# kristi700/ViT-SSL

Hardware: AMD Instinct MI355X
Metric: images_per_sec (higher is better)
Workload: dtype bf16; 1 GPU; ViT-B/16 SimMIM 224x224 mask 0.6 dropout 0.1 AdamW, batch 256/GPU; global_batch=256, parallelism=dp1

## Files before the change

__graft_entry__.py:

```python
import os
import subprocess
import sys
from concurrent.futures import ThreadPoolExecutor

ROOT = os.path.dirname(os.path.abspath(__file__))
PKG = os.path.join(ROOT, "vit-ssl_amd")
CSRC = os.path.join(PKG, "csrc")
OUT_DIR = os.path.join(PKG, "vitssl_hip")
LIB = os.path.join(OUT_DIR, "libvitssl_hip.so")
SOURCES = ["error.cpp", "gemm_nt.hip", "gemm_tn.hip", "layernorm.hip", "attention.hip", "attention_long.hip", "elementwise.hip", "dino.hip", "augment.hip", "transforms.hip", "metrics.hip", "classify.hip", "fp8.hip"]
HIPCC = os.environ.get("HIPCC", "/opt/rocm/bin/hipcc")
PER_FILE_FLAGS = {"augment.hip": ["-ffp-contract=off"], "transforms.hip": ["-ffp-contract=off"]}
FLAGS = ["--offload-arch=gfx950", "-O3", "-fPIC", "-std=c++17", "-Wno-unused-result"] + os.environ.get("VITSSL_HIPCC_FLAGS", "").split()


def _needs_rebuild(target, deps):
    if not os.path.exists(target):
        return True
    t = os.path.getmtime(target)
    return any(os.path.getmtime(d) > t for d in deps if os.path.exists(d))


def build(force: bool = False, verbose: bool = False) -> None:
    srcs = [os.path.join(CSRC, s) for s in SOURCES if os.path.exists(os.path.join(CSRC, s))]
    hdrs = [os.path.join(CSRC, "common.h"), os.path.join(CSRC, "attention_tiles.h"), os.path.join(CSRC, "attention_bwd.h"),
            os.path.join(CSRC, "resample_taps.h"),
            os.path.join(ROOT, "include", "vitssl_hip.h"), os.path.join(ROOT, "include", "vitssl_transforms.h"),
            os.path.join(ROOT, "include", "vitssl_metrics.h"), os.path.join(ROOT, "include", "vitssl_classify.h")]
    objdir = os.path.join(CSRC, "build")
    os.makedirs(objdir, exist_ok=True)

    def compile_one(src):
        obj = os.path.join(objdir, os.path.basename(src) + ".o")
        if force or _needs_rebuild(obj, [src] + hdrs + [os.path.abspath(__file__)]):
            cmd = [HIPCC] + FLAGS + PER_FILE_FLAGS.get(os.path.basename(src), []) + ["-x", "hip", "-c", src, "-o", obj]
            r = subprocess.run(cmd, capture_output=True, text=True)
            if r.returncode != 0:
                raise RuntimeError(f"hipcc failed for {src}:\n{r.stderr[-4000:]}")
            if verbose and r.stderr.strip():
                print(r.stderr, file=sys.stderr)
        return obj

    with ThreadPoolExecutor(max_workers=4) as ex:
        objs = list(ex.map(compile_one, srcs))
    if force or _needs_rebuild(LIB, objs):
        cmd = [HIPCC, "--offload-arch=gfx950", "-shared", "-fPIC", "-o", LIB] + objs
        r = subprocess.run(cmd, capture_output=True, text=True)
        if r.returncode != 0:
            raise RuntimeError(f"link failed:\n{r.stderr[-4000:]}")
    if PKG not in sys.path:
        sys.path.insert(0, PKG)
    import vitssl_hip
    vitssl_hip.lib()


def smoke() -> None:
    for p in (ROOT, PKG):
        if p not in sys.path:
            sys.path.insert(0, p)
    import torch
    from vitssl_hip import smoke_check
# ... 8 lines not shown
```

vit-ssl_amd/csrc/elementwise.hip:

```cpp
#include "common.h"

namespace {

constexpr int EW_THREADS = 256;

inline unsigned ew_grid(long long work_items) {
  long long g = (work_items + EW_THREADS - 1) / EW_THREADS;
  if (g < 1) g = 1;
  return (unsigned)g;
}

__global__ void dropout_mask_kernel(unsigned char* keep, long long ngroups, DropKey dk) {
  const long long grp = (long long)blockIdx.x * blockDim.x + threadIdx.x;
  if (grp >= ngroups) return;
  float m[4];
  drop_mult4(dk, (unsigned)grp, m);
  uchar4 o;
  o.x = m[0] != 0.f; o.y = m[1] != 0.f; o.z = m[2] != 0.f; o.w = m[3] != 0.f;
  if (dk.thr == 0) o = make_uchar4(1, 1, 1, 1);
  *(uchar4*)(keep + 4 * grp) = o;
}

template <bool GATHER, typename OutT>
__global__ void patchify_kernel(const float* __restrict__ img, const int* __restrict__ idx, OutT* __restrict__ out,
                                long long nrows, int C, int H, int W, int P) {
  const int gw = W / P, gh = H / P;
  const int pd4 = C * P * P / 4;
  const long long t = (long long)blockIdx.x * blockDim.x + threadIdx.x;
  if (t >= nrows * pd4) return;
  const long long r = t / pd4;
  const int f = (int)(t - r * pd4) * 4;
  const long long m = GATHER ? (long long)idx[r] : r;
  const long long b = m / (gh * gw);
  const int pi = (int)(m - b * gh * gw);
  const int py = pi / gw, px = pi - py * gw;
  const int c = f / (P * P);
  const int kh = (f - c * P * P) / P;
  const int kw = f - c * P * P - kh * P;
  const f32x4 v = *(const f32x4*)(img + ((b * C + c) * H + (py * P + kh)) * (long long)W + px * P + kw);
  if constexpr (sizeof(OutT) == 2) {
    u32x2 w = {pack_bf2(v[0], v[1]), pack_bf2(v[2], v[3])};
    *(u32x2*)((bf16_t*)out + r * (4LL * pd4) + f) = w;
  } else {
    *(f32x4*)((float*)out + r * (4LL * pd4) + f) = v;
  }
}

__global__ void gather_rows_bf16_kernel(const float* __restrict__ x, const int* __restrict__ idx, bf16_t* __restrict__ out,
                                        int n_idx, int cols) {
  const int c4n = cols >> 2;
  const long long t = (long long)blockIdx.x * blockDim.x + threadIdx.x;
  if (t >= (long long)n_idx * c4n) return;
  const int i = (int)(t / c4n);
  const int c = (int)(t - (long long)i * c4n) * 4;
  const f32x4 v = *(const f32x4*)(x + (long long)idx[i] * cols + c);
  u32x2 w = {pack_bf2(v[0], v[1]), pack_bf2(v[2], v[3])};
  *(u32x2*)(out + (long long)i * cols + c) = w;
}

__global__ void scatter_rows_f32_kernel(const bf16_t* __restrict__ src, const int* __restrict__ inv, float* __restrict__ g,
                                        long long rows, int cols) {
  const int c4n = cols >> 2;
  const long long t = (long long)blockIdx.x * blockDim.x + threadIdx.x;
  if (t >= rows * c4n) return;
  const long long r = t / c4n;
  const int c = (int)(t - r * c4n) * 4;
  const int i = inv[r];
  f32x4 v = {0.f, 0.f, 0.f, 0.f};
  if (i >= 0) {
    const u32x2 w = *(const u32x2*)(src + (long long)i * cols + c);
    v = f32x4{bf_lo(w[0]), bf_hi(w[0]), bf_lo(w[1]), bf_hi(w[1])};
  }
  *(f32x4*)(g + r * cols + c) = v;
}

__global__ void gather_cls_kernel(const float* __restrict__ x, float* __restrict__ out, int B, int T, int D) {
  const int d4n = D >> 2;
  const long long t = (long long)blockIdx.x * blockDim.x + threadIdx.x;
  if (t >= (long long)B * d4n) return;
  const int b = (int)(t / d4n);
// ... 125 lines not shown
__global__ void cast_bf16_kernel(const float* __restrict__ src, bf16_t* __restrict__ dst, long long n) {
  const long long n4 = n >> 2;
  for (long long i = (long long)blockIdx.x * blockDim.x + threadIdx.x; i < n4; i += (long long)gridDim.x * blockDim.x) {
    const f32x4 v = *(const f32x4*)(src + 4 * i);
    u32x2 w = {pack_bf2(v[0], v[1]), pack_bf2(v[2], v[3])};
    *(u32x2*)(dst + 4 * i) = w;
  }
  if (blockIdx.x == 0 && threadIdx.x < (n & 3)) dst[(n4 << 2) + threadIdx.x] = f2bf(src[(n4 << 2) + threadIdx.x]);
}

__global__ void cast_transpose_kernel(const float* __restrict__ src, bf16_t* __restrict__ dst, bf16_t* __restrict__ dst_t,
                                      int R, int C) {
  __shared__ bf16_t tile[64][66];
  const int r0 = blockIdx.y * 64, c0 = blockIdx.x * 64;
  const int tx = threadIdx.x & 63, ty = threadIdx.x >> 6;
  for (int rr = ty; rr < 64; rr += 4) {
    const int r = r0 + rr, c = c0 + tx;
    bf16_t h = 0;
    if (r < R && c < C) {
      h = f2bf(src[(long long)r * C + c]);
      if (dst) dst[(long long)r * C + c] = h;
    }
    tile[rr][tx] = h;
  }
  __syncthreads();
  if (dst_t) {
    for (int cc = ty; cc < 64; cc += 4) {
      const int c = c0 + cc, r = r0 + tx;
      if (c < C && r < R) dst_t[(long long)c * R + r] = tile[tx][cc];
    }
  }
}

__global__ void cast_transpose_batch_kernel(const vitssl_cast_job_t* __restrict__ jobs, const int* __restrict__ tile_start,
                                            int njobs) {
  __shared__ bf16_t tile[64][66];
  const int b = blockIdx.x;
  int lo = 0, hi = njobs;
  while (hi - lo > 1) {
    const int mid = (lo + hi) >> 1;
    if (tile_start[mid] <= b) lo = mid; else hi = mid;
  }
  const vitssl_cast_job_t j = jobs[lo];
  const int t = b - tile_start[lo];
  const int tx_n = (j.C + 63) >> 6;
  const int r0 = (t / tx_n) * 64, c0 = (t % tx_n) * 64;
  const int R = j.R, C = j.C;
  bf16_t* dst = (bf16_t*)j.dst;
  bf16_t* dst_t = (bf16_t*)j.dst_t;
  const int tx = threadIdx.x & 63, ty = threadIdx.x >> 6;
  for (int rr = ty; rr < 64; rr += 4) {
    const int r = r0 + rr, c = c0 + tx;
    bf16_t h = 0;
    if (r < R && c < C) {
      h = f2bf(j.src[(long long)r * C + c]);
      if (dst) dst[(long long)r * C + c] = h;
    }
    tile[rr][tx] = h;
  }
  __syncthreads();
  if (dst_t) {
    for (int cc = ty; cc < 64; cc += 4) {
      const int c = c0 + cc, r = r0 + tx;
      if (c < C && r < R) dst_t[(long long)c * R + r] = tile[tx][cc];
    }
  }
}

__global__ void adamw_kernel(float* __restrict__ p, const float* __restrict__ g, float* __restrict__ m, float* __restrict__ v,
                             long long n, float lr, float b1, float b2, float eps, float wd, float bc1, float bc2_sqrt,
                             float gscale) {
  const long long n4 = n >> 2;
  const float step_size = lr / bc1;
  for (long long i = (long long)blockIdx.x * blockDim.x + threadIdx.x; i < n4; i += (long long)gridDim.x * blockDim.x) {
    f32x4 pv = *(const f32x4*)(p + 4 * i);
    const f32x4 gv = *(const f32x4*)(g + 4 * i) * gscale;
    f32x4 mv = *(const f32x4*)(m + 4 * i);
    f32x4 vv = *(const f32x4*)(v + 4 * i);
    pv *= (1.f - lr * wd);
    mv = mv * b1 + gv * (1.f - b1);
    vv = vv * b2 + gv * gv * (1.f - b2);
#pragma unroll
// ... 130 lines not shown
  VS_CHECK_ARG(keep && rows > 0 && cols > 0 && cols % 4 == 0, "dropout_mask: cols must be a multiple of 4");
  VS_CHECK_ARG((unsigned long long)rows * (unsigned long long)cols < (1ull << 34), "dropout_mask: the stream's group counter is 32 bits (rows * cols < 2^34)");
  const long long ng = rows * cols / 4;
  hipLaunchKernelGGL(dropout_mask_kernel, dim3(ew_grid(ng)), dim3(EW_THREADS), 0, (hipStream_t)stream, keep, ng, make_drop_key(d));
  VS_CHECK_LAUNCH("dropout_mask");
  return VITSSL_OK;
}

static int check_patch_args(const char* who, int B, int C, int H, int W, int P) {
  VS_CHECK_ARG(B > 0 && C > 0 && P > 0 && P % 4 == 0, "%s: patch size %d must be a positive multiple of 4", who, P);
  VS_CHECK_ARG(H % P == 0 && W % P == 0, "%s: image %dx%d not divisible by patch %d", who, H, W, P);
  return VITSSL_OK;
}

extern "C" int vitssl_patchify_bf16(const float* img, void* patches, int B, int C, int H, int W, int P, void* stream) {
  VS_CHECK_ARG(img && patches, "patchify: null pointer");
  if (int rc = check_patch_args("patchify", B, C, H, W, P)) return rc;
  const long long nrows = (long long)B * (H / P) * (W / P);
  const long long work = nrows * (C * P * P / 4);
  hipLaunchKernelGGL((patchify_kernel<false, bf16_t>), dim3(ew_grid(work)), dim3(EW_THREADS), 0, (hipStream_t)stream, img,
                     (const int*)nullptr, (bf16_t*)patches, nrows, C, H, W, P);
  VS_CHECK_LAUNCH("patchify");
  return VITSSL_OK;
}

extern "C" int vitssl_gather_patches_f32(const float* img, const int32_t* idx, float* out, int n_idx, int C, int H, int W,
                                         int P, void* stream) {
  VS_CHECK_ARG(img && idx && out && n_idx > 0, "gather_patches: null pointer / empty");
  if (int rc = check_patch_args("gather_patches", 1, C, H, W, P)) return rc;
  const long long work = (long long)n_idx * (C * P * P / 4);
  hipLaunchKernelGGL((patchify_kernel<true, float>), dim3(ew_grid(work)), dim3(EW_THREADS), 0, (hipStream_t)stream, img, idx,
                     out, (long long)n_idx, C, H, W, P);
  VS_CHECK_LAUNCH("gather_patches");
  return VITSSL_OK;
}

extern "C" int vitssl_gather_rows_bf16(const float* x, const int32_t* idx, void* out, int n_idx, int cols, void* stream) {
  VS_CHECK_ARG(x && idx && out && n_idx > 0 && cols > 0 && cols % 4 == 0, "gather_rows: bad args");
  hipLaunchKernelGGL(gather_rows_bf16_kernel, dim3(ew_grid((long long)n_idx * (cols / 4))), dim3(EW_THREADS), 0,
                     (hipStream_t)stream, x, idx, (bf16_t*)out, n_idx, cols);
  VS_CHECK_LAUNCH("gather_rows");
  return VITSSL_OK;
}

extern "C" int vitssl_scatter_rows_f32(const void* src_bf16, const int32_t* inv, float* g, int64_t rows, int cols, void* stream) {
  VS_CHECK_ARG(src_bf16 && inv && g && rows > 0 && cols > 0 && cols % 4 == 0, "scatter_rows: bad args");
  hipLaunchKernelGGL(scatter_rows_f32_kernel, dim3(ew_grid(rows * (cols / 4))), dim3(EW_THREADS), 0, (hipStream_t)stream,
                     (const bf16_t*)src_bf16, inv, g, (long long)rows, cols);
  VS_CHECK_LAUNCH("scatter_rows");
  return VITSSL_OK;
}

extern "C" int vitssl_gather_cls_f32(const float* x, float* out, int B, int T, int D, void* stream) {
  VS_CHECK_ARG(x && out && B > 0 && T > 0 && D > 0 && D % 4 == 0, "gather_cls: bad args");
  hipLaunchKernelGGL(gather_cls_kernel, dim3(ew_grid((long long)B * (D / 4))), dim3(EW_THREADS), 0, (hipStream_t)stream, x, out, B, T, D);
  VS_CHECK_LAUNCH("gather_cls");
  return VITSSL_OK;
}

extern "C" int vitssl_scatter_cls_f32(const float* gcls, float* g, int B, int T, int D, void* stream) {
  VS_CHECK_ARG(gcls && g && B > 0 && T > 0 && D > 0 && D % 4 == 0, "scatter_cls: bad args");
  hipLaunchKernelGGL(scatter_cls_kernel, dim3(ew_grid((long long)B * T * (D / 4))), dim3(EW_THREADS), 0, (hipStream_t)stream, gcls, g, B, T, D);
  VS_CHECK_LAUNCH("scatter_cls");
  return VITSSL_OK;
}

// ... 71 lines not shown
}

extern "C" int vitssl_colsum_bf16(const void* x_bf16, float* out, int64_t rows, int cols, float* workspace, int64_t workspace_floats,
                                  void* stream) {
  VS_CHECK_ARG(x_bf16 && out && rows > 0 && cols > 0 && cols % 4 == 0, "colsum_bf16: bad args");
  int splits = (int)((rows + 127) / 128);
  if (splits > 512) splits = 512;
  float* parts = vs_sum_parts(workspace, workspace_floats, (long long)splits * cols, rows, cols, "colsum_bf16");
  if (!parts) return VITSSL_ERR_ARG;
  hipLaunchKernelGGL(colsum_bf16_kernel, dim3((cols / 4 + EW_THREADS - 1) / EW_THREADS, splits), dim3(EW_THREADS), 0,
                     (hipStream_t)stream, (const bf16_t*)x_bf16, parts, (long long)rows, cols);
  VS_CHECK_LAUNCH("colsum_bf16");
  return vs_reduce_parts(out, parts, splits, cols, cols, (hipStream_t)stream);
}

extern "C" int vitssl_cast_bf16(const float* src, void* dst, int64_t n, void* stream) {
  VS_CHECK_ARG(src && dst && n > 0, "cast_bf16: bad args");
  hipLaunchKernelGGL(cast_bf16_kernel, dim3(stream_grid(n / 4)), dim3(EW_THREADS), 0, (hipStream_t)stream, src, (bf16_t*)dst, (long long)n);
  VS_CHECK_LAUNCH("cast_bf16");
  return VITSSL_OK;
}

extern "C" int vitssl_cast_transpose_bf16(const float* src, void* dst, void* dst_t, int R, int C, void* stream) {
  VS_CHECK_ARG(src && (dst || dst_t) && R > 0 && C > 0, "cast_transpose: bad args");
  hipLaunchKernelGGL(cast_transpose_kernel, dim3((C + 63) / 64, (R + 63) / 64), dim3(EW_THREADS), 0, (hipStream_t)stream, src,
                     (bf16_t*)dst, (bf16_t*)dst_t, R, C);
  VS_CHECK_LAUNCH("cast_transpose");
  return VITSSL_OK;
}

extern "C" int vitssl_cast_transpose_batch(const vitssl_cast_job_t* jobs, const int* tile_start, int njobs, int total_tiles,
                                           void* stream) {
  VS_CHECK_ARG(jobs && tile_start && njobs > 0 && total_tiles > 0, "cast_transpose_batch: bad args");
  hipLaunchKernelGGL(cast_transpose_batch_kernel, dim3(total_tiles), dim3(EW_THREADS), 0, (hipStream_t)stream, jobs, tile_start,
                     njobs);
  VS_CHECK_LAUNCH("cast_transpose_batch");
  return VITSSL_OK;
}

extern "C" int vitssl_adamw(float* p, const float* g, float* m, float* v, int64_t n, float lr, float beta1, float beta2,
                            float eps, float wd, int step, float gscale, void* stream) {
  VS_CHECK_ARG(p && g && m && v && n > 0 && step >= 1, "adamw: bad args");
  const double bc1 = 1.0 - pow((double)beta1, (double)step);
  const double bc2 = 1.0 - pow((double)beta2, (double)step);
  hipLaunchKernelGGL(adamw_kernel, dim3(stream_grid(n / 4)), dim3(EW_THREADS), 0, (hipStream_t)stream, p, g, m, v, (long long)n, lr,
                     beta1, beta2, eps, wd, (float)bc1, (float)sqrt(bc2), gscale);
  VS_CHECK_LAUNCH("adamw");
  return VITSSL_OK;
}

extern "C" int vitssl_ema(float* teacher, const float* student, int64_t n, float m, void* stream) {
  VS_CHECK_ARG(teacher && student && n > 0, "ema: bad args");
  hipLaunchKernelGGL(ema_kernel, dim3(stream_grid(n / 4)), dim3(EW_THREADS), 0, (hipStream_t)stream, teacher, student, (long long)n, m);
  VS_CHECK_LAUNCH("ema");
  return VITSSL_OK;
}
```

vit-ssl_amd/vit_core/ssl/simmim/model.py:

```python
import torch
from torch import nn
from torch.autograd import Function

from ... import _runtime as R
from ..._runtime import BF16, F32, L, ops
from ...encoder_block import EncoderBlock
from .masking import draw_mask, mask_indices_np


class _SimMIMRuntime:

    def __init__(self, model: "SimMIMViT", device):
        self.model = model
        self.device = device
        C, H, W = model.input_shape
        self.P = model.patch_size
        self.C, self.H, self.W = C, H, W
        self.N = (H // self.P) * (W // self.P)
        self.Pd = C * self.P * self.P
        self.D = model.embed_dim
        self.store = R.FlatStore(model, device)
        st = self.store
        prefixes = [f"encoder_blocks.{i}." for i in range(len(model.encoder_blocks))]
        self.stack = R.EncoderStack(st, prefixes, self.D, model.num_heads, model.mlp_dim, model.dropout_p)
        st.register_weight("proj", lambda: st.view("projection.weight", (self.D, self.Pd)), transposed_too=False)
        st.register_weight("head", lambda: st.view("simmim_head.weight", (self.Pd, self.D)))
        self.ws = R.Workspace()
        self.rec = None
        self.save_gen = 0

    def valid_for(self, device) -> bool:
        return device == self.device and self.store.is_attached()

    def embed(self, x, mask_d, tag=""):
        st, ws = self.store, self.ws
        B = x.shape[0]
        M = B * self.N
        patches = ws.get(tag + "patches", (M, self.Pd), BF16, x.device)
        ops.patchify_bf16(x, patches, self.P)
        x0 = ws.get(tag + "x0", (M, self.D), F32, x.device)
        ops.gemm_nt(patches, st.w("proj"), x0, L.EPI_EMBED, bias=st.view("projection.bias"),
                    embed=(mask_d, st.view("mask_token") if mask_d is not None else None,
                           st.view("positional_embedding", (self.N, self.D)), self.N, self.N, 0))
        return x0, patches

    def prepare_mask(self, mask_cpu, dev):
        idx, inv, mflat = mask_indices_np(mask_cpu.contiguous())
        M, Mm = inv.size, idx.size
        key = (M, Mm, str(dev))
        if getattr(self, "_stage_key", None) != key:
            nslots = 4
            self._stage = [dict(idx=torch.empty(Mm, dtype=torch.int32).pin_memory(),
                                inv=torch.empty(M, dtype=torch.int32).pin_memory(),
                                mask=torch.empty(M, dtype=torch.uint8).pin_memory(), ev=None) for _ in range(nslots)]
            self._stage_dev = [dict(idx=torch.empty(Mm, dtype=torch.int32, device=dev),
                                    inv=torch.empty(M, dtype=torch.int32, device=dev),
                                    mask=torch.empty(M, dtype=torch.uint8, device=dev)) for _ in range(nslots)]
            self._stage_pos = 0
            self._stage_key = key
        k = self._stage_pos % len(self._stage)
        self._stage_pos += 1
        slot, d = self._stage[k], self._stage_dev[k]
        if slot["ev"] is not None:
            slot["ev"].synchronize()
        slot["idx"].numpy()[:] = idx
        slot["inv"].numpy()[:] = inv
        slot["mask"].numpy()[:] = mflat
        for name in ("idx", "inv", "mask"):
            d[name].copy_(slot[name], non_blocking=True)
        slot["ev"] = torch.cuda.Event()
        slot["ev"].record(torch.cuda.current_stream())
        return d["idx"], d["inv"], d["mask"]

    def forward(self, x, training: bool, save: bool, mask_cpu=None, prepared=None):
        st, ws = self.store, self.ws
        if x.dim() != 4 or tuple(x.shape[1:]) != (self.C, self.H, self.W):
            raise L.VitsslError(f"SimMIMViT: expected input [B,{self.C},{self.H},{self.W}], got {tuple(x.shape)}")
        self.stack.check_tokens(self.N)
        x = R.as_f32(x)
        B = x.shape[0]
        M = B * self.N
        st.refresh_weights()
        dev = x.device
        if prepared is None:
            if mask_cpu is None:
                mask_cpu = draw_mask(B, self.N, self.model.mask_ratio)
            prepared = self.prepare_mask(mask_cpu, dev)
        seed = R.next_seed() if (training and self.stack.p > 0) else 0
        idx_d, inv_d, mask_d = prepared
        Mm = idx_d.numel()

        targets = torch.empty(Mm, self.Pd, dtype=F32, device=dev)
        if Mm == 0:
            if save:
                self.save_gen += 1
                self.rec = dict(B=B, M=M, Mm=0)
            return torch.empty(0, self.Pd, dtype=F32, device=dev), targets, mask_d.view(B, self.N, 1).bool()
        ops.gather_patches_f32(x, idx_d, targets, self.P)
        tag = "" if save else "tmp."
        x0, patches = self.embed(x, mask_d, tag)
        xL, _ = self.stack.forward(x0, B, self.N, training, seed, save=save, slot="a")
        sel = ws.get(tag + "sel", (Mm, self.D), BF16, dev)
        ops.gather_rows_bf16(xL, idx_d, sel)
        pred = torch.empty(Mm, self.Pd, dtype=F32, device=dev)
        ops.gemm_nt(sel, st.w("head"), pred, L.EPI_F32, bias=st.view("simmim_head.bias"))
        if save:
            self.save_gen += 1
            self.rec = dict(B=B, M=M, Mm=Mm, idx=idx_d, inv=inv_d, mask=mask_d, patches=patches, sel=sel)
        return pred, targets, mask_d.view(B, self.N, 1).bool()

    def backward(self, dpred_bf16, reducer=None):
        st, ws, rec = self.store, self.ws, self.rec
        B, M, Mm = rec["B"], rec["M"], rec["Mm"]
        if Mm == 0:
            if reducer is not None:
                reducer.ready(0, st.gflat.numel())
            return
        dev = dpred_bf16.device
        gv = st.gview
        ops.colsum_bf16(dpred_bf16, gv("simmim_head.bias"))
        ops.gemm_tn(dpred_bf16, rec["sel"], gv("simmim_head.weight", (self.Pd, self.D)))
        dsel = ws.get("dsel", (Mm, self.D), BF16, dev)
        ops.gemm_nt(dpred_bf16, st.w("head.T"), dsel, L.EPI_BF16)
        g = ws.get("g", (M, self.D), F32, dev)
        ops.scatter_rows_f32(dsel, rec["inv"], g)
        if reducer is not None:
            reducer.ready(*st.span("simmim_head.weight", "simmim_head.bias"))
        g = self.stack.backward(g, slot="a", reducer=reducer)
        dproj = ws.get("dproj", (M, self.D), BF16, dev)
        ops.embed_bwd(g, rec["mask"], dproj, gv("positional_embedding", (self.N, self.D)), gv("mask_token"),
                      gv("projection.bias"), None, B, self.N, 0, self.D)
        ops.gemm_tn(dproj, rec["patches"], gv("projection.weight", (self.D, self.Pd)))
        if reducer is not None:
# ... 126 lines not shown
```

vit-ssl_amd/vitssl_hip/_lib.py:

```python
import ctypes as C
import os
import re

_HERE = os.path.dirname(os.path.abspath(__file__))
LIB_PATH = os.environ.get("VITSSL_LIB") or os.path.join(_HERE, "libvitssl_hip.so")
HEADER_PATH = os.path.normpath(os.path.join(_HERE, "..", "..", "include", "vitssl_hip.h"))
TRANSFORMS_HEADER_PATH = os.path.normpath(os.path.join(_HERE, "..", "..", "include", "vitssl_transforms.h"))
METRICS_HEADER_PATH = os.path.normpath(os.path.join(_HERE, "..", "..", "include", "vitssl_metrics.h"))
CLASSIFY_HEADER_PATH = os.path.normpath(os.path.join(_HERE, "..", "..", "include", "vitssl_classify.h"))


class VitsslError(RuntimeError):
    pass


class Dropout(C.Structure):
    _fields_ = [("p", C.c_float), ("site", C.c_uint32), ("seed", C.c_uint64)]


class Embed(C.Structure):
    _fields_ = [("mask", C.c_void_p), ("mask_token", C.c_void_p), ("pos", C.c_void_p),
                ("tokens", C.c_int), ("out_tokens", C.c_int), ("tok_offset", C.c_int)]


class TnJob(C.Structure):
    _fields_ = [("A", C.c_void_p), ("B", C.c_void_p), ("C", C.c_void_p), ("N1", C.c_int), ("N2", C.c_int)]


class Fp8TnJob(C.Structure):
    _fields_ = [("A8", C.c_void_p), ("B8", C.c_void_p), ("C", C.c_void_p), ("N1", C.c_int), ("N2", C.c_int),
                ("alpha", C.c_void_p), ("alpha2", C.c_void_p)]


class Gemm(C.Structure):
    _fields_ = [("A", C.c_void_p), ("B", C.c_void_p), ("M", C.c_int64), ("N", C.c_int), ("K", C.c_int),
                ("epilogue", C.c_int), ("bias", C.c_void_p), ("aux", C.c_void_p), ("out0", C.c_void_p),
                ("out1", C.c_void_p), ("colsum", C.c_void_p), ("drop", Dropout), ("embed", Embed),
                ("workspace", C.c_void_p), ("workspace_floats", C.c_int64)]


class Fp8Gemm(C.Structure):
# ... 41 lines not shown
    "vitssl_cast_bf16": [_vp, _vp, _i64, _vp],
    "vitssl_cast_transpose_bf16": [_vp, _vp, _vp, _i, _i, _vp],
    "vitssl_cast_transpose_batch": [_vp, _vp, _i, _i, _vp],
    "vitssl_bicubic_resize_fwd": [_vp, _vp, _i, _i, _i, _i, _i, _vp],
    "vitssl_bicubic_resize_bwd": [_vp, _vp, _i, _i, _i, _i, _i, _vp],
    "vitssl_aug_resized_crop_u8": [_vp, _vp, _vp, _vp, _i, _i, _i, _i, _vp],
    "vitssl_aug_color_u8": [_vp, _vp, _vp, _i, _i, _vp],
    "vitssl_aug_blur_to_tensor": [_vp, _vp, _vp, _i, _i, _i, _vp],
    "vitssl_adamw": [_vp, _vp, _vp, _vp, _i64, _f, _f, _f, _f, _f, _i, _f, _vp],
    "vitssl_ema": [_vp, _vp, _i64, _f, _vp],
    "vitssl_rownorm_fwd": [_vp, _vp, _vp, _i64, _i, _vp],
    "vitssl_rownorm_bwd": [_vp, _vp, _vp, _vp, _i64, _i, _vp],
    "vitssl_weightnorm_fold": [_vp, _vp, _vp, _vp, _i, _i, _vp],
    "vitssl_weightnorm_bwd": [_vp, _vp, _vp, _vp, _vp, _vp, _i, _i, _vp],
    "vitssl_dino_loss": [_vp, _vp, _vp, _vp, _i64, _vp, _vp, _i, _i, _i, _i, _f, _f, _f, _vp],
    "vitssl_colsum_f32": [_vp, _vp, _i64, _i, _vp],
    "vitssl_center_ema": [_vp, _vp, _i, _f, _f, _vp],
    "vitssl_set_reserved_cus": [_i],
}

PROTOTYPES_TRANSFORMS = {
    "vitssl_tf_resized_crop_to_tensor": [_vp, _vp, _vp, _i, _i, _i, _i, _i, _vp],
}

PROTOTYPES_METRICS = {
    "vitssl_recon_metrics": [_vp, _vp, _vp, _i64, _i, _i, _vp, _i64, _vp],
    "vitssl_dino_stats": [_vp, _vp, _vp, _vp, _i, _i, _i, _i, _vp, _i64, _vp],
}

PROTOTYPES_CLASSIFY = {
    "vitssl_classify_loss": [_vp, _vp, _i, _i, _i, C.c_double, _i64, _f, _vp, _vp, _i, _vp, _vp, _vp, _vp, _vp, _i64, _vp],
}

_lib = None


def header_symbols():
    with open(HEADER_PATH) as f:
        txt = f.read()
    return sorted(set(re.findall(r"\b(vitssl_[a-z0-9_]+)\s*\(", txt)))


def transforms_header_symbols():
    with open(TRANSFORMS_HEADER_PATH) as f:
        txt = re.sub(r"/\*.*?\*/", "", f.read(), flags=re.S)
    return sorted(set(re.findall(r"\b(vitssl_[a-z0-9_]+)\s*\(", txt)))


def metrics_header_symbols():
    with open(METRICS_HEADER_PATH) as f:
        txt = re.sub(r"/\*.*?\*/", "", f.read(), flags=re.S)
    return sorted(set(re.findall(r"\b(vitssl_[a-z0-9_]+)\s*\(", txt)))


def classify_header_symbols():
    with open(CLASSIFY_HEADER_PATH) as f:
        txt = re.sub(r"/\*.*?\*/", "", f.read(), flags=re.S)
    return sorted(set(re.findall(r"\b(vitssl_[a-z0-9_]+)\s*\(", txt)))


def lib():
    global _lib
    if _lib is not None:
        return _lib
    if not os.path.exists(LIB_PATH):
        raise VitsslError(
            f"{LIB_PATH} not found: the HIP library is not built. Run `python __graft_entry__.py` "
            "(or __graft_entry__.build()). There is no CPU fallback for the vit_core hot path.")
    import torch
    l = C.CDLL(LIB_PATH)
    l.vitssl_last_error.restype = C.c_char_p
    l.vitssl_last_error.argtypes = []
    l.vitssl_version.restype = C.c_int
    l.vitssl_version.argtypes = []
    if l.vitssl_version() != ABI_VERSION:
        raise VitsslError(f"{LIB_PATH} implements C-ABI version {l.vitssl_version()}, these bindings expect {ABI_VERSION}: "
                          "rebuild it (python __graft_entry__.py)")
    l.vitssl_gemm_tn_workspace_floats.restype = C.c_int64
    l.vitssl_gemm_tn_workspace_floats.argtypes = [C.c_int64, C.c_int, C.c_int]
    l.vitssl_gemm_tn_batch_workspace_floats.restype = C.c_int64
    l.vitssl_gemm_tn_batch_workspace_floats.argtypes = [C.POINTER(TnJob), C.c_int, C.c_int64]
    l.vitssl_gemm_fp8_tn_batch_workspace_floats.restype = C.c_int64
    l.vitssl_gemm_fp8_tn_batch_workspace_floats.argtypes = [C.POINTER(Fp8TnJob), C.c_int, C.c_int64]
    l.vitssl_gemm_fp8_tn_workspace_floats.restype = C.c_int64
    l.vitssl_gemm_fp8_tn_workspace_floats.argtypes = [C.c_int64, C.c_int, C.c_int]
    l.vitssl_dino_loss_workspace_floats.restype = C.c_int64
    l.vitssl_dino_loss_workspace_floats.argtypes = [C.c_int, C.c_int, C.c_int]
    l.vitssl_sum_workspace_floats.restype = C.c_int64
    l.vitssl_sum_workspace_floats.argtypes = [C.c_int64, C.c_int]
    l.vitssl_embed_bwd_workspace_floats.restype = C.c_int64
    l.vitssl_embed_bwd_workspace_floats.argtypes = [C.c_int, C.c_int, C.c_int, C.c_int]
    for getter in ("vitssl_get_reserved_cus", "vitssl_debug_last_nt_grid", "vitssl_debug_last_attn_fwd_grid"):
        getattr(l, getter).restype = C.c_int
        getattr(l, getter).argtypes = []
    l.vitssl_debug_tf_tile_rows.restype = C.c_int
    l.vitssl_debug_tf_tile_rows.argtypes = [C.c_int, C.c_int, C.c_int, C.c_int]
    l.vitssl_recon_metrics_workspace_floats.restype = C.c_int64
    l.vitssl_recon_metrics_workspace_floats.argtypes = [C.c_int64, C.c_int, C.c_int]
    l.vitssl_dino_stats_workspace_floats.restype = C.c_int64
    l.vitssl_dino_stats_workspace_floats.argtypes = [C.c_int, C.c_int, C.c_int, C.c_int]
    l.vitssl_classify_loss_workspace_floats.restype = C.c_int64
    l.vitssl_classify_loss_workspace_floats.argtypes = [C.c_int, C.c_int]
    for name, args in (list(PROTOTYPES.items()) + list(PROTOTYPES_TRANSFORMS.items()) + list(PROTOTYPES_METRICS.items())
                       + list(PROTOTYPES_CLASSIFY.items())):
        fn = getattr(l, name)
        fn.restype = C.c_int
        fn.argtypes = args
    _lib = l
    return l


def call(name, *args):
    l = lib()
    rc = getattr(l, name)(*args)
    if rc != 0:
        raise VitsslError(f"{name} failed ({rc}): {l.vitssl_last_error().decode()}")
```

vit-ssl_amd/vitssl_hip/ops.py:

```python
import ctypes as C

import torch

from . import _lib as L
from ._lib import Dropout, Embed, Fp8Gemm, Gemm, call

BF16 = torch.bfloat16
F32 = torch.float32
FP8 = torch.float8_e4m3fn


def _stream():
    return C.c_void_p(torch.cuda.current_stream().cuda_stream)


def _chk(t, dtype, name, shape=None):
    if t is None:
        raise L.VitsslError(f"{name}: tensor is None")
    if not t.is_cuda:
        raise L.VitsslError(f"{name}: expected a CUDA (HIP) tensor, got {t.device}; there is no CPU fallback")
    if t.device.index != torch.cuda.current_device():
        raise L.VitsslError(f"{name}: tensor lives on {t.device} but the current device is cuda:{torch.cuda.current_device()}; "
                            "call torch.cuda.set_device (one process per GPU) before using the engine")
    if t.dtype != dtype:
        raise L.VitsslError(f"{name}: expected dtype {dtype}, got {t.dtype}")
    if not t.is_contiguous():
        raise L.VitsslError(f"{name}: tensor must be contiguous")
    if shape is not None and tuple(t.shape) != tuple(shape):
        raise L.VitsslError(f"{name}: expected shape {tuple(shape)}, got {tuple(t.shape)}")
    return C.c_void_p(t.data_ptr())


def _opt(t, dtype, name, shape=None):
    return C.c_void_p(0) if t is None else _chk(t, dtype, name, shape)


def make_dropout(p=0.0, seed=0, site=0):
    return Dropout(float(p), int(site) & 0xFFFFFFFF, int(seed) & 0xFFFFFFFFFFFFFFFF)


NO_DROP = make_dropout()

PROFILE = None


def _prof_begin():
    if PROFILE is None:
        return None
    ev = torch.cuda.Event(enable_timing=True)
    ev.record(torch.cuda.current_stream())
    return ev


def _prof_end(ev0, label, flops, nbytes=0):
    if ev0 is None:
        return
    ev1 = torch.cuda.Event(enable_timing=True)
    ev1.record(torch.cuda.current_stream())
    PROFILE.append((label, flops, ev0, ev1, nbytes))


def dropout_mask(rows, cols, drop, device):
    keep = torch.empty(rows, cols, dtype=torch.uint8, device=device)
    call("vitssl_dropout_mask", _chk(keep, torch.uint8, "keep"), rows, cols, drop, _stream())
    return keep


def layernorm_fwd(x, gamma, beta, y, mean, rstd, eps=1e-5):
    rows, cols = x.shape
    ev = _prof_begin()
    call("vitssl_layernorm_fwd", _chk(x, F32, "x"), _chk(gamma, F32, "gamma", (cols,)), _chk(beta, F32, "beta", (cols,)),
         _chk(y, BF16, "y", (rows, cols)), _chk(mean, F32, "mean", (rows,)), _chk(rstd, F32, "rstd", (rows,)),
         rows, cols, float(eps), _stream())
    _prof_end(ev, "ln_fwd", 0.0, rows * (6 * cols + 8))
# ... 249 lines not shown
        call("vitssl_attn_bwd_fp8", _chk(qkv, BF16, "qkv", (B * N, 3 * H * dh)), _chk(out, BF16, "out", (B * N, H * dh)),
             _chk(dout, BF16, "dout", (B * N, H * dh)), _chk(lse, F32, "lse", (B, H, N)), _opt(dqkv, BF16, "dqkv", (B * N, 3 * H * dh)),
             _chk(dqkv_fp8, FP8, "dqkv_fp8", (B * N, 3 * H * dh)), _scalar(scale, "scale"), _scalar(amax, "amax"), B, N, H, dh, _stream())
    else:
        _attn_bwd(qkv, out, dout, lse, dqkv, delta_ws, B, N, H, dh)
    _prof_end(ev, f"attn_bwd B{B} N{N} H{H}", 8.0 * B * H * N * N * dh)


def _attn_bwd(qkv, out, dout, lse, dqkv, delta_ws, B, N, H, dh):
    call("vitssl_attn_bwd", _chk(qkv, BF16, "qkv", (B * N, 3 * H * dh)), _chk(out, BF16, "out", (B * N, H * dh)),
         _chk(dout, BF16, "dout", (B * N, H * dh)), _chk(lse, F32, "lse", (B, H, N)),
         _chk(dqkv, BF16, "dqkv", (B * N, 3 * H * dh)), _chk(delta_ws, F32, "delta_ws", (B, H, N)), B, N, H, dh, _stream())


def patchify_bf16(img, patches, P):
    B, Cc, H, W = img.shape
    call("vitssl_patchify_bf16", _chk(img, F32, "img"), _chk(patches, BF16, "patches", (B * (H // P) * (W // P), Cc * P * P)),
         B, Cc, H, W, P, _stream())


def gather_patches_f32(img, idx, out, P):
    B, Cc, H, W = img.shape
    n = idx.numel()
    call("vitssl_gather_patches_f32", _chk(img, F32, "img"), _chk(idx, torch.int32, "idx"), _chk(out, F32, "out", (n, Cc * P * P)),
         n, Cc, H, W, P, _stream())


def gather_rows_bf16(x, idx, out):
    rows, cols = x.shape
    n = idx.numel()
    call("vitssl_gather_rows_bf16", _chk(x, F32, "x"), _chk(idx, torch.int32, "idx"), _chk(out, BF16, "out", (n, cols)), n, cols, _stream())


def scatter_rows_f32(src, inv, g):
    rows, cols = g.shape
    call("vitssl_scatter_rows_f32", _chk(src, BF16, "src"), _chk(inv, torch.int32, "inv", (rows,)), _chk(g, F32, "g"), rows, cols, _stream())


def gather_cls_f32(x, out, B, T, D):
    call("vitssl_gather_cls_f32", _chk(x, F32, "x", (B * T, D)), _chk(out, F32, "out", (B, D)), B, T, D, _stream())


def scatter_cls_f32(gcls, g, B, T, D):
    call("vitssl_scatter_cls_f32", _chk(gcls, F32, "gcls", (B, D)), _chk(g, F32, "g", (B * T, D)), B, T, D, _stream())


def embed_bwd(dtok, mask, dproj, dpos, dmask_token, dbias, dcls, B, tokens, tok_offset, D):
    T_out = tokens + tok_offset
    wsn = int(L.lib().vitssl_embed_bwd_workspace_floats(B, tokens, tok_offset, D))
    ws = _tn_workspace(dtok.device, wsn)
    call("vitssl_embed_bwd", _chk(dtok, F32, "dtok", (B * T_out, D)), _opt(mask, torch.uint8, "mask", (B * tokens,)),
         _chk(dproj, BF16, "dproj", (B * tokens, D)), _opt(dpos, F32, "dpos", (T_out, D)),
         _opt(dmask_token, F32, "dmask_token", (D,)), _opt(dbias, F32, "dbias", (D,)), _opt(dcls, F32, "dcls", (D,)),
         B, tokens, tok_offset, D, C.c_void_p(ws.data_ptr()), ws.numel(), _stream())


def l1_loss(pred, target, loss_sum, dpred=None, gscale=0.0):
    n = pred.numel()
    call("vitssl_l1_loss", _chk(pred, F32, "pred"), _chk(target, F32, "target", pred.shape), _chk(loss_sum, F32, "loss_sum", (1,)),
         _opt(dpred, BF16, "dpred", pred.shape), float(gscale), n, *_sum_ws(pred.device, n, 1), _stream())


def cross_entropy(logits, labels, loss_sum, dlogits=None, gscale=0.0):
    B, Cn = logits.shape
    call("vitssl_cross_entropy", _chk(logits, F32, "logits"), _chk(labels, torch.int64, "labels", (B,)),
         _chk(loss_sum, F32, "loss_sum", (1,)), _opt(dlogits, BF16, "dlogits", (B, Cn)), float(gscale), B, Cn, _stream())
# ... 260 lines not shown
```

Baseline: 7879 images/s.

## Fuse patchify with target gather, vectorize cast-transpose, pack mask uploads

```diff
diff --git a/__graft_entry__.py b/__graft_entry__.py
--- a/__graft_entry__.py
+++ b/__graft_entry__.py
@@ -26,7 +26,8 @@
     hdrs = [os.path.join(CSRC, "common.h"), os.path.join(CSRC, "attention_tiles.h"), os.path.join(CSRC, "attention_bwd.h"),
             os.path.join(CSRC, "resample_taps.h"),
             os.path.join(ROOT, "include", "vitssl_hip.h"), os.path.join(ROOT, "include", "vitssl_transforms.h"),
-            os.path.join(ROOT, "include", "vitssl_metrics.h"), os.path.join(ROOT, "include", "vitssl_classify.h")]
+            os.path.join(ROOT, "include", "vitssl_metrics.h"), os.path.join(ROOT, "include", "vitssl_classify.h"),
+            os.path.join(ROOT, "include", "vitssl_step_glue.h")]
     objdir = os.path.join(CSRC, "build")
     os.makedirs(objdir, exist_ok=True)
 
diff --git a/include/vitssl_step_glue.h b/include/vitssl_step_glue.h
--- /dev/null
+++ b/include/vitssl_step_glue.h
@@ -0,0 +1,16 @@
+#ifndef VITSSL_STEP_GLUE_H
+#define VITSSL_STEP_GLUE_H
+
+#include <stdint.h>
+
+#ifdef __cplusplus
+extern "C" {
+#endif
+
+int vitssl_patchify_targets(const float* img, const int32_t* inv, void* patches, float* targets, int n_idx, int B, int C,
+                            int H, int W, int P, void* stream);
+
+#ifdef __cplusplus
+}
+#endif
+#endif
diff --git a/vit-ssl_amd/csrc/elementwise.hip b/vit-ssl_amd/csrc/elementwise.hip
--- a/vit-ssl_amd/csrc/elementwise.hip
+++ b/vit-ssl_amd/csrc/elementwise.hip
@@ -1,4 +1,5 @@
 #include "common.h"
+#include "../../include/vitssl_step_glue.h"
 
 namespace {
 
@@ -46,6 +47,27 @@
   }
 }
 
+__global__ void patchify_targets_kernel(const float* __restrict__ img, const int* __restrict__ inv, bf16_t* __restrict__ patches,
+                                        float* __restrict__ targets, long long nrows, int n_idx, int C, int H, int W, int P) {
+  const int gw = W / P, gh = H / P;
+  const int pd4 = C * P * P / 4;
+  const long long t = (long long)blockIdx.x * blockDim.x + threadIdx.x;
+  if (t >= nrows * pd4) return;
+  const long long m = t / pd4;
+  const int f = (int)(t - m * pd4) * 4;
+  const long long b = m / (gh * gw);
+  const int pi = (int)(m - b * gh * gw);
+  const int py = pi / gw, px = pi - py * gw;
+  const int c = f / (P * P);
+  const int kh = (f - c * P * P) / P;
+  const int kw = f - c * P * P - kh * P;
+  const f32x4 v = *(const f32x4*)(img + ((b * C + c) * H + (py * P + kh)) * (long long)W + px * P + kw);
+  u32x2 w = {pack_bf2(v[0], v[1]), pack_bf2(v[2], v[3])};
+  *(u32x2*)(patches + m * (4LL * pd4) + f) = w;
+  const int i = inv[m];
+  if (i >= 0 && i < n_idx) *(f32x4*)(targets + i * (4LL * pd4) + f) = v;
+}
+
 __global__ void gather_rows_bf16_kernel(const float* __restrict__ x, const int* __restrict__ idx, bf16_t* __restrict__ out,
                                         int n_idx, int cols) {
   const int c4n = cols >> 2;
@@ -237,9 +259,10 @@
   }
 }
 
+template <bool VEC>
 __global__ void cast_transpose_batch_kernel(const vitssl_cast_job_t* __restrict__ jobs, const int* __restrict__ tile_start,
                                             int njobs) {
-  __shared__ bf16_t tile[64][66];
+  __shared__ __attribute__((aligned(16))) unsigned smem[64 * 66 / 2];
   const int b = blockIdx.x;
   int lo = 0, hi = njobs;
   while (hi - lo > 1) {
@@ -253,6 +276,38 @@
   const int R = j.R, C = j.C;
   bf16_t* dst = (bf16_t*)j.dst;
   bf16_t* dst_t = (bf16_t*)j.dst_t;
+  if constexpr (VEC) {
+    const unsigned long long align = (unsigned long long)j.src | (unsigned long long)j.dst | (unsigned long long)j.dst_t;
+    if (r0 + 64 <= R && c0 + 64 <= C && ((R | C) & 7) == 0 && (align & 15) == 0) {
+      const int cj = threadIdx.x & 7, kk = threadIdx.x >> 3;
+      const float* p = j.src + (long long)(r0 + 2 * kk) * C + c0 + 8 * cj;
+      const f32x4 a0 = *(const f32x4*)p, a1 = *(const f32x4*)(p + 4);
+      const f32x4 b0 = *(const f32x4*)(p + C), b1 = *(const f32x4*)(p + C + 4);
+      if (dst) {
+        bf16_t* q = dst + (long long)(r0 + 2 * kk) * C + c0 + 8 * cj;
+        *(u32x4*)q = u32x4{pack_bf2(a0[0], a0[1]), pack_bf2(a0[2], a0[3]), pack_bf2(a1[0], a1[1]), pack_bf2(a1[2], a1[3])};
+        *(u32x4*)(q + C) = u32x4{pack_bf2(b0[0], b0[1]), pack_bf2(b0[2], b0[3]), pack_bf2(b1[0], b1[1]), pack_bf2(b1[2], b1[3])};
+      }
+      if (dst_t) {
+        const int ks = kk ^ (cj << 2);
+#pragma unroll
+        for (int i = 0; i < 4; ++i) {
+          smem[(8 * cj + i) * 32 + ks] = pack_bf2(a0[i], b0[i]);
+          smem[(8 * cj + 4 + i) * 32 + ks] = pack_bf2(a1[i], b1[i]);
+        }
+        __syncthreads();
+        const int jr = threadIdx.x & 7;
+#pragma unroll
+        for (int pass = 0; pass < 2; ++pass) {
+          const int c = (threadIdx.x >> 3) + 32 * pass;
+          const u32x4 w = *(const u32x4*)(smem + c * 32 + ((4 * jr) ^ (((c >> 3) & 7) << 2)));
+          *(u32x4*)(dst_t + (long long)(c0 + c) * R + r0 + 8 * jr) = w;
+        }
+      }
+      return;
+    }
+  }
+  bf16_t(*tile)[66] = (bf16_t(*)[66])smem;
   const int tx = threadIdx.x & 63, ty = threadIdx.x >> 6;
   for (int rr = ty; rr < 64; rr += 4) {
     const int r = r0 + rr, c = c0 + tx;
@@ -449,6 +504,18 @@
   hipLaunchKernelGGL((patchify_kernel<true, float>), dim3(ew_grid(work)), dim3(EW_THREADS), 0, (hipStream_t)stream, img, idx,
                      out, (long long)n_idx, C, H, W, P);
   VS_CHECK_LAUNCH("gather_patches");
+  return VITSSL_OK;
+}
+
+extern "C" int vitssl_patchify_targets(const float* img, const int32_t* inv, void* patches, float* targets, int n_idx, int B, int C,
+                                       int H, int W, int P, void* stream) {
+  VS_CHECK_ARG(img && inv && patches && n_idx >= 0 && (targets || n_idx == 0), "patchify_targets: null pointer");
+  if (int rc = check_patch_args("patchify_targets", B, C, H, W, P)) return rc;
+  const long long nrows = (long long)B * (H / P) * (W / P);
+  const long long work = nrows * (C * P * P / 4);
+  hipLaunchKernelGGL(patchify_targets_kernel, dim3(ew_grid(work)), dim3(EW_THREADS), 0, (hipStream_t)stream, img, inv,
+                     (bf16_t*)patches, targets, nrows, n_idx, C, H, W, P);
+  VS_CHECK_LAUNCH("patchify_targets");
   return VITSSL_OK;
 }
 
@@ -586,8 +653,13 @@
 extern "C" int vitssl_cast_transpose_batch(const vitssl_cast_job_t* jobs, const int* tile_start, int njobs, int total_tiles,
                                            void* stream) {
   VS_CHECK_ARG(jobs && tile_start && njobs > 0 && total_tiles > 0, "cast_transpose_batch: bad args");
-  hipLaunchKernelGGL(cast_transpose_batch_kernel, dim3(total_tiles), dim3(EW_THREADS), 0, (hipStream_t)stream, jobs, tile_start,
-                     njobs);
+  static VsEnvInt step_glue;
+  if (step_glue.get("VITSSL_STEP_GLUE", 1) != 0)
+    hipLaunchKernelGGL(cast_transpose_batch_kernel<true>, dim3(total_tiles), dim3(EW_THREADS), 0, (hipStream_t)stream, jobs,
+                       tile_start, njobs);
+  else
+    hipLaunchKernelGGL(cast_transpose_batch_kernel<false>, dim3(total_tiles), dim3(EW_THREADS), 0, (hipStream_t)stream, jobs,
+                       tile_start, njobs);
   VS_CHECK_LAUNCH("cast_transpose_batch");
   return VITSSL_OK;
 }
diff --git a/vit-ssl_amd/vit_core/ssl/simmim/model.py b/vit-ssl_amd/vit_core/ssl/simmim/model.py
--- a/vit-ssl_amd/vit_core/ssl/simmim/model.py
+++ b/vit-ssl_amd/vit_core/ssl/simmim/model.py
@@ -32,12 +32,15 @@
     def valid_for(self, device) -> bool:
         return device == self.device and self.store.is_attached()
 
-    def embed(self, x, mask_d, tag=""):
+    def embed(self, x, mask_d, tag="", targets=None, inv_d=None):
         st, ws = self.store, self.ws
         B = x.shape[0]
         M = B * self.N
         patches = ws.get(tag + "patches", (M, self.Pd), BF16, x.device)
-        ops.patchify_bf16(x, patches, self.P)
+        if targets is not None:
+            ops.patchify_targets(x, inv_d, patches, targets, self.P)
+        else:
+            ops.patchify_bf16(x, patches, self.P)
         x0 = ws.get(tag + "x0", (M, self.D), F32, x.device)
         ops.gemm_nt(patches, st.w("proj"), x0, L.EPI_EMBED, bias=st.view("projection.bias"),
                     embed=(mask_d, st.view("mask_token") if mask_d is not None else None,
@@ -47,6 +50,8 @@
     def prepare_mask(self, mask_cpu, dev):
         idx, inv, mflat = mask_indices_np(mask_cpu.contiguous())
         M, Mm = inv.size, idx.size
+        if ops.STEP_GLUE:
+            return self._prepare_mask_packed(idx, inv, mflat, dev)
         key = (M, Mm, str(dev))
         if getattr(self, "_stage_key", None) != key:
             nslots = 4
@@ -72,6 +77,37 @@
         slot["ev"].record(torch.cuda.current_stream())
         return d["idx"], d["inv"], d["mask"]
 
+    def _prepare_mask_packed(self, idx, inv, mflat, dev):
+        M, Mm = inv.size, idx.size
+        key = (M, Mm, str(dev))
+        if getattr(self, "_pack_key", None) != key:
+            up = lambda n: (n + 255) // 256 * 256
+            o_idx = up(4 * M)
+            o_mask = o_idx + up(4 * Mm)
+            total = o_mask + up(M)
+            self._pack = []
+            for _ in range(4):
+                h = torch.empty(total, dtype=torch.uint8).pin_memory()
+                d = torch.empty(total, dtype=torch.uint8, device=dev)
+                hn = h.numpy()
+                self._pack.append(dict(h=h, d=d, ev=None,
+                                       h_inv=hn[:4 * M].view("<i4"), h_idx=hn[o_idx:o_idx + 4 * Mm].view("<i4"), h_mask=hn[o_mask:o_mask + M],
+                                       d_inv=d[:4 * M].view(torch.int32), d_idx=d[o_idx:o_idx + 4 * Mm].view(torch.int32),
+                                       d_mask=d[o_mask:o_mask + M]))
+            self._pack_pos = 0
+            self._pack_key = key
+        slot = self._pack[self._pack_pos % len(self._pack)]
+        self._pack_pos += 1
+        if slot["ev"] is not None:
+            slot["ev"].synchronize()
+        slot["h_inv"][:] = inv
+        slot["h_idx"][:] = idx
+        slot["h_mask"][:] = mflat
+        slot["d"].copy_(slot["h"], non_blocking=True)
+        slot["ev"] = torch.cuda.Event()
+        slot["ev"].record(torch.cuda.current_stream())
+        return slot["d_idx"], slot["d_inv"], slot["d_mask"]
+
     def forward(self, x, training: bool, save: bool, mask_cpu=None, prepared=None):
         st, ws = self.store, self.ws
         if x.dim() != 4 or tuple(x.shape[1:]) != (self.C, self.H, self.W):
@@ -96,9 +132,12 @@
                 self.save_gen += 1
                 self.rec = dict(B=B, M=M, Mm=0)
             return torch.empty(0, self.Pd, dtype=F32, device=dev), targets, mask_d.view(B, self.N, 1).bool()
-        ops.gather_patches_f32(x, idx_d, targets, self.P)
         tag = "" if save else "tmp."
-        x0, patches = self.embed(x, mask_d, tag)
+        if ops.STEP_GLUE:
+            x0, patches = self.embed(x, mask_d, tag, targets, inv_d)
+        else:
+            ops.gather_patches_f32(x, idx_d, targets, self.P)
+            x0, patches = self.embed(x, mask_d, tag)
         xL, _ = self.stack.forward(x0, B, self.N, training, seed, save=save, slot="a")
         sel = ws.get(tag + "sel", (Mm, self.D), BF16, dev)
         ops.gather_rows_bf16(xL, idx_d, sel)
diff --git a/vit-ssl_amd/vitssl_hip/_lib.py b/vit-ssl_amd/vitssl_hip/_lib.py
--- a/vit-ssl_amd/vitssl_hip/_lib.py
+++ b/vit-ssl_amd/vitssl_hip/_lib.py
@@ -7,6 +7,7 @@
 HEADER_PATH = os.path.normpath(os.path.join(_HERE, "..", "..", "include", "vitssl_hip.h"))
 TRANSFORMS_HEADER_PATH = os.path.normpath(os.path.join(_HERE, "..", "..", "include", "vitssl_transforms.h"))
 METRICS_HEADER_PATH = os.path.normpath(os.path.join(_HERE, "..", "..", "include", "vitssl_metrics.h"))
+STEP_GLUE_HEADER_PATH = os.path.normpath(os.path.join(_HERE, "..", "..", "include", "vitssl_step_glue.h"))
 CLASSIFY_HEADER_PATH = os.path.normpath(os.path.join(_HERE, "..", "..", "include", "vitssl_classify.h"))
 
 
@@ -114,6 +115,10 @@
     "vitssl_classify_loss": [_vp, _vp, _i, _i, _i, C.c_double, _i64, _f, _vp, _vp, _i, _vp, _vp, _vp, _vp, _vp, _i64, _vp],
 }
 
+PROTOTYPES_STEP_GLUE = {
+    "vitssl_patchify_targets": [_vp, _vp, _vp, _vp, _i, _i, _i, _i, _i, _i, _vp],
+}
+
 _lib = None
 
 
@@ -137,6 +142,12 @@
 
 def classify_header_symbols():
     with open(CLASSIFY_HEADER_PATH) as f:
+        txt = re.sub(r"/\*.*?\*/", "", f.read(), flags=re.S)
+    return sorted(set(re.findall(r"\b(vitssl_[a-z0-9_]+)\s*\(", txt)))
+
+
+def step_glue_header_symbols():
+    with open(STEP_GLUE_HEADER_PATH) as f:
         txt = re.sub(r"/\*.*?\*/", "", f.read(), flags=re.S)
     return sorted(set(re.findall(r"\b(vitssl_[a-z0-9_]+)\s*\(", txt)))
 
@@ -184,7 +195,7 @@
     l.vitssl_classify_loss_workspace_floats.restype = C.c_int64
     l.vitssl_classify_loss_workspace_floats.argtypes = [C.c_int, C.c_int]
     for name, args in (list(PROTOTYPES.items()) + list(PROTOTYPES_TRANSFORMS.items()) + list(PROTOTYPES_METRICS.items())
-                       + list(PROTOTYPES_CLASSIFY.items())):
+                       + list(PROTOTYPES_CLASSIFY.items()) + list(PROTOTYPES_STEP_GLUE.items())):
         fn = getattr(l, name)
         fn.restype = C.c_int
         fn.argtypes = args
diff --git a/vit-ssl_amd/vitssl_hip/ops.py b/vit-ssl_amd/vitssl_hip/ops.py
--- a/vit-ssl_amd/vitssl_hip/ops.py
+++ b/vit-ssl_amd/vitssl_hip/ops.py
@@ -1,4 +1,5 @@
 import ctypes as C
+import os
 
 import torch
 
@@ -40,6 +41,16 @@
 
 
 NO_DROP = make_dropout()
+
+
+def _env_flag(name, default):
+    try:
+        return int(os.environ.get(name, default), 0) != 0
+    except ValueError:
+        return bool(default)
+
+
+STEP_GLUE = _env_flag("VITSSL_STEP_GLUE", "1")
 
 PROFILE = None
 
@@ -355,6 +366,14 @@
     call("vitssl_gather_rows_bf16", _chk(x, F32, "x"), _chk(idx, torch.int32, "idx"), _chk(out, BF16, "out", (n, cols)), n, cols, _stream())
 
 
+def patchify_targets(img, inv, patches, targets, P):
+    B, Cc, H, W = img.shape
+    M, Pd = B * (H // P) * (W // P), Cc * P * P
+    n = targets.shape[0]
+    call("vitssl_patchify_targets", _chk(img, F32, "img"), _chk(inv, torch.int32, "inv", (M,)), _chk(patches, BF16, "patches", (M, Pd)),
+         _chk(targets, F32, "targets", (n, Pd)) if n else C.c_void_p(0), n, B, Cc, H, W, P, _stream())
+
+
 def scatter_rows_f32(src, inv, g):
     rows, cols = g.shape
     call("vitssl_scatter_rows_f32", _chk(src, BF16, "src"), _chk(inv, torch.int32, "inv", (rows,)), _chk(g, F32, "g"), rows, cols, _stream())
```

Measured after the change: 7905 images/s (median of 6 runs). About the same (+0.3%).
